# instance-based-loc/instance-based-loc

Hardware: AMD Instinct MI355X
Metric: query-frames localized/sec (embed+match+register) (higher is better)
Workload: dtype f16 (ViT MFMA operands, f32 accumulate) / f32+f64 (match, registration); 1 GPU; T: dinov2_vitb14 crops 224^2 (Q=7), 10000-instance memory (E=4), FPFH+RANSAC+coloured ICP on 5000-pt clouds, whole-memory evaluate; synthetic objects of extent U[0.15, 0.6] m on a 2.50 m grid (SURVEY 8d's U[0.2, 1.5] m re-scoped: its 5 000 points are too sparse to survive the radius-outlier removal); memory_instances=10000, points_per_object=5000, resident_feature_bytes_per_point=264, parallelism=frames-dp1+memory-replicated

## Files before the change

### instance-based-loc_amd/csrc/reg_api.hip

```cpp
#pragma clang fp contract(off)
#include <hip/hip_runtime.h>

#include <hipcub/hipcub.hpp>

#include <cctype>
#include <climits>
#include <cmath>
#include <cstdlib>
#include <cstring>
#include <string>
#include <vector>

#include "ibloc.h"
#include "reg_common.h"

#ifndef KNN_CELLS_NORMAL
#define KNN_CELLS_NORMAL 3.0
#endif
#ifndef KNN_CELLS_FEATURE
#define KNN_CELLS_FEATURE 5.0
#endif

#ifndef KNN_TILE_NORMAL
#define KNN_TILE_NORMAL 4
#endif
#ifndef KNN_TILE_FEATURE
#define KNN_TILE_FEATURE 2
#endif

int ibl_launch_normals(ibl_reg_ctx* ctx, const BatchGrid& g, const float4* pts, const int* seg_off, int n, double radius, int max_nn, float4* normals,
                       int* status, hipStream_t s);
int ibl_launch_fpfh(ibl_reg_ctx* ctx, const BatchGrid& g, const float4* pts, const float4* normals, const int* seg_off, int n, double radius, int max_nn,
                    unsigned char* spfh, int* nbr_idx, float* nbr_d2, int* nbr_cnt, float* fpfh, int matching_order, int* status,
                    hipStream_t s);
int ibl_launch_radius_count(const BatchGrid& g, const float4* pts, const int* seg_off, int n, double radius, int nb_points,
                            unsigned char* keep, hipStream_t s);

bool ibl_normals_fpfh_fusable(const ibl_reg_ctx* ctx, double radius_normal, int max_nn_normal, double radius_feature, int max_nn_feature);
int ibl_launch_normals_fpfh(ibl_reg_ctx* ctx, const BatchGrid& g, const float4* pts, const int* seg_off, int n, double radius_normal,
                            int max_nn_normal, double radius_feature, int max_nn_feature, float4* normals, unsigned char* spfh, int* nbr_idx,
                            float* nbr_d2, int* nbr_cnt, float* fpfh, int matching_order, int* status, hipStream_t s);
int ibl_launch_color_grad(ibl_reg_ctx* ctx, const BatchGrid& g, const float4* pts, const float4* normals, const int* seg_off, int q0, int q1, double radius,
                          int max_nn, float4* grad, int* status, hipStream_t s);

static int ibl_bbox_to_host(ibl_reg_ctx* ctx, const float4* P, const int* seg_off_dev, int n_seg, float* bbox_host, hipStream_t s) {
    if (n_seg <= 0) return IBL_OK;
    ArenaMark m(ctx);
    float* bbox;
    IBL_ARENA(bbox, float, (int64_t)n_seg * 6 + 6);
    int st = ibl_launch_bbox(P, seg_off_dev, n_seg, bbox, s);
    if (st) return st;
    IBL_HIP_CHECK(hipMemcpyAsync(bbox_host, bbox, sizeof(float) * 6 * (size_t)n_seg, hipMemcpyDeviceToHost, s));
    IBL_HIP_CHECK(hipStreamSynchronize(s));
    return IBL_OK;
}

struct DiagSwitch {
    const char* name;
    int RegDiag::*field;
    int lo = INT_MIN, hi = INT_MAX;
    bool auto0 = false;
};
static const DiagSwitch DIAG_SWITCHES[] = {
    {"knn_safety", nullptr},
    {"knn_rho", &RegDiag::knn_rho, 1, 4},
    {"knn_noguess", &RegDiag::knn_noguess},
    {"knn_debug", &RegDiag::knn_debug},
    {"feat_unfused", &RegDiag::feat_unfused},
    {"feat_valu", &RegDiag::feat_valu},
    {"feat_cand_cap", &RegDiag::feat_cand_cap, 1, INT_MAX, true},
    {"feat_p1_stride", &RegDiag::feat_p1_stride, 1},
    {"spfh_f64", &RegDiag::spfh_f64},
    {"spfh_qcap", &RegDiag::spfh_qcap, 1, INT_MAX, true},
    {"spfh_stats", &RegDiag::spfh_stats},
    {"eval_fullscan", &RegDiag::eval_fullscan},
    {"timing", &RegDiag::timing},
};

static const DiagSwitch* find_diag(const char* name) {
    for (const DiagSwitch& d : DIAG_SWITCHES)
        if (name && strcmp(name, d.name) == 0) return &d;
    return nullptr;
}

extern "C" int ibl_reg_ctx_set_diag(ibl_reg_ctx* ctx, const char* name, double value) {
    const DiagSwitch* d = find_diag(name);
    if (!ctx || !d || !std::isfinite(value)) return ibl_set_error(IBL_ERR_ARG, "ibl_reg_ctx_set_diag: null context, unknown switch or non-finite value");
    if (!d->field) ctx->diag.knn_safety = value;
    else if (d->auto0 && value == 0) ctx->diag.*d->field = 0;
    else ctx->diag.*d->field = (int)std::min(std::max(value, (double)d->lo), (double)d->hi);
    return IBL_OK;
}

extern "C" int ibl_reg_ctx_get_diag(const ibl_reg_ctx* ctx, const char* name, double* value) {
    const DiagSwitch* d = find_diag(name);
    if (!ctx || !d || !value) return ibl_set_error(IBL_ERR_ARG, "ibl_reg_ctx_get_diag: null argument or unknown switch");
    *value = d->field ? (double)(ctx->diag.*d->field) : ctx->diag.knn_safety;
    return IBL_OK;
}

extern "C" int ibl_reg_ctx_create(ibl_reg_ctx** out, int64_t arena_bytes) {
    if (!out || arena_bytes < (1 << 20)) return ibl_set_error(IBL_ERR_ARG, "ibl_reg_ctx_create: bad argument");
    ibl_reg_ctx* c = new ibl_reg_ctx();
    IBL_HIP_CHECK(hipGetDevice(&c->device));
    hipError_t e = hipMalloc(reinterpret_cast<void**>(&c->base), (size_t)arena_bytes);
    if (e != hipSuccess) {
        delete c;
        return ibl_set_error(IBL_ERR_HIP, "ibl_reg_ctx_create: hipMalloc(%lld) failed: %s", (long long)arena_bytes, hipGetErrorString(e));
    }
    c->size = arena_bytes;
    c->d_status = reinterpret_cast<int*>(c->base);
    c->used = 256;
    e = hipMemset(c->base, 0, 256);
    if (e != hipSuccess) { (void)hipFree(c->base); delete c; return ibl_set_error(IBL_ERR_HIP, "ibl_reg_ctx_create: memset failed"); }
    c->pin_size = 32 << 20;
    if (hipHostMalloc(reinterpret_cast<void**>(&c->pin), (size_t)c->pin_size, hipHostMallocDefault) != hipSuccess) { c->pin = nullptr; c->pin_size = 0; }
    for (const DiagSwitch& d : DIAG_SWITCHES) {
        std::string var = "IBL_";
        for (const char* p = d.name; *p; ++p) var += (char)toupper((unsigned char)*p);
        if (const char* v = getenv(var.c_str())) (void)ibl_reg_ctx_set_diag(c, d.name, atof(v));
    }
    *out = c;
    return IBL_OK;
}

extern "C" int ibl_reg_ctx_destroy(ibl_reg_ctx* ctx) {
    if (!ctx) return IBL_OK;
    (void)hipFree(ctx->base);
    if (ctx->pin) (void)hipHostFree(ctx->pin);
    delete ctx;
    return IBL_OK;
}

extern "C" int ibl_reg_ctx_reset(ibl_reg_ctx* ctx) {
    if (!ctx) return ibl_set_error(IBL_ERR_ARG, "ibl_reg_ctx_reset: null context");
    ctx->used = 256;
    return IBL_OK;
}

extern "C" int64_t ibl_reg_ctx_high_water(const ibl_reg_ctx* ctx) { return ctx ? ctx->high_water : -1; }

extern "C" int ibl_reg_ctx_status(ibl_reg_ctx* ctx, int clear) {
    if (!ctx) return -1;
    int h = 0;
    if (hipMemcpy(&h, ctx->d_status, sizeof(int), hipMemcpyDeviceToHost) != hipSuccess) return -1;
    if (clear) (void)hipMemset(ctx->d_status, 0, sizeof(int));
    return h;
}

static int check_seg(const int32_t* seg_off_host, int n_seg, const char* who) {
    if (!seg_off_host || n_seg < 0) return ibl_set_error(IBL_ERR_ARG, "%s: bad segment table", who);
    if (seg_off_host[0] != 0) return ibl_set_error(IBL_ERR_ARG, "%s: seg_off[0] must be 0", who);
    for (int s = 0; s < n_seg; ++s)
        if (seg_off_host[s + 1] < seg_off_host[s]) return ibl_set_error(IBL_ERR_ARG, "%s: seg_off must be non-decreasing", who);
// ... 306 lines not shown
```

### instance-based-loc_amd/csrc/reg_common.h

```cpp
#pragma once
#include <hip/hip_runtime.h>

#include <cstdint>

#include "ibl_common.h"

struct SegGrid {
    float minx, miny, minz, inv;
    int nx, ny, nz;
    int cell_base;
};

struct BatchGrid {
    const SegGrid* seg;
    const int* cell_start;
    const float4* sorted_pts;
    const int* order;
    int n_seg;
    const int* tile_base;
    const int* tile_seg;
    int n_tiles;
    int ts;
};

#define FM_P1_STRIDE 2

struct RegDiag {
    double knn_safety = 1.1;
    int knn_rho = 3;
    int knn_noguess = 0, knn_debug = 0;
    int feat_unfused = 0, feat_valu = 0, feat_cand_cap = 0;
    int feat_p1_stride = FM_P1_STRIDE;
    int spfh_f64 = 0, spfh_qcap = 0, spfh_stats = 0;
    int eval_fullscan = 0;
    int timing = 0;
};

struct ibl_reg_ctx {
    RegDiag diag;
    unsigned char* base = nullptr;
    int64_t size = 0;
    int64_t used = 0;
    int64_t high_water = 0;
    int device = 0;
    int* d_status = nullptr;
    unsigned char* pin = nullptr;
    int64_t pin_size = 0;
    int64_t pin_used = 0;
};

int ibl_stage_upload(ibl_reg_ctx* ctx, void* dst_dev, const void* src_host, int64_t bytes, hipStream_t s);
static inline void ibl_stage_reset(ibl_reg_ctx* ctx) { ctx->pin_used = 0; }

struct ArenaMark {
    ibl_reg_ctx* ctx;
    int64_t mark;
    explicit ArenaMark(ibl_reg_ctx* c) : ctx(c), mark(c->used) {}
    ~ArenaMark() { ctx->used = mark; }
};

template <typename T>
static inline T* arena_alloc(ibl_reg_ctx* ctx, int64_t count, bool* ok) {
    int64_t bytes = ibl_align_up(count * (int64_t)sizeof(T), 256);
    if (bytes < 256) bytes = 256;
    if (ctx->used + bytes > ctx->size) {
        *ok = false;
        return nullptr;
    }
    T* p = reinterpret_cast<T*>(ctx->base + ctx->used);
    ctx->used += bytes;
    if (ctx->used > ctx->high_water) ctx->high_water = ctx->used;
    return p;
}

#define IBL_ARENA(ptr, type, count)                                                                  \
    do {                                                                                             \
        bool _ok = true;                                                                             \
        ptr = arena_alloc<type>(ctx, (count), &_ok);                                                 \
        if (!_ok)                                                                                    \
            return ibl_set_error(IBL_ERR_ARENA, "device arena exhausted (%lld of %lld bytes used, need %lld more) at %s:%d", \
                                 (long long)ctx->used, (long long)ctx->size,                         \
                                 (long long)((count) * (int64_t)sizeof(type)), __FILE__, __LINE__);  \
    } while (0)

#define IBL_ERR_ARENA (-5)
#define IBL_ERR_OVERFLOW (-6)

#define IBL_ST_GRID_OVERFLOW 1
#define IBL_ST_KNN_SLOWPATH 2
#define IBL_ST_FEAT_OVERFLOW 4
#define IBL_ST_RANSAC_OVERFLOW 8
#define IBL_ST_FEAT_REDONE 16
#define IBL_ST_RANSAC_REDONE 32

int ibl_build_batch_grid(ibl_reg_ctx* ctx, const float4* pts, const int* seg_off_dev, const int* seg_off_host, int n_seg,
                         float cell, int64_t max_cells, bool collapse, BatchGrid* out, hipStream_t s);
int ibl_build_batch_grid_bounded(ibl_reg_ctx* ctx, const float4* pts, const int* seg_off_dev, const int* seg_off_host, int n_seg,
                                 float cell, int64_t cells_bound, BatchGrid* out, hipStream_t s);
int ibl_build_tile_grid(ibl_reg_ctx* ctx, const float4* pts, const int* seg_off_dev, const int* seg_off_host, int n_seg,
                        const float* bbox_host, double radius, int max_nn, int ts, int64_t max_cells, BatchGrid* out, hipStream_t s);

int ibl_launch_bbox(const float4* pts, const int* seg_off_dev, int n_seg, float* bbox_dev, hipStream_t s);

struct FeatSources { const float4* normals[3]; const float* fpfh[3]; const float4* grad[3]; const unsigned short* split[3]; const float* norm[3]; };
struct FeatPair { int qkind, qsrc, qcnt, dkind, dsrc, dcnt, out, pad; };

int ibl_feat_search_mfma(ibl_reg_ctx* ctx, const FeatPair* d_pairs, int n_pairs, int max_q, const FeatSources& src, int* pair_idx,
                         float* pair_d2, const int* need_pos, const int* need_list, int out0, int64_t out_count, bool* overflow,
                         hipStream_t s);

int ibl_features_on_batch(ibl_reg_ctx* ctx, const float4* P, const int* seg_off_dev, const int* seg_off_host, int n_seg, const float* bbox_host, double voxel_size,
                          double grad_radius, int gq0, int gq1, float4* normals, float* fpfh, unsigned short* fpfh_split, float* fpfh_norm,
                          float4* grad, hipStream_t s);

#ifdef __HIPCC__
__device__ __constant__ const float FM_MU[33] = {87.f, 46.f, 101.f, 26.f, 28.f, 17.f, 26.f, 26.f, 17.f, 14.f, 21.f, 7.f, 14.f, 19.f, 7.f, 8.f, 14.f,
                                                 6.f,  8.f,  13.f,  6.f,  5.f,  11.f, 6.f,  5.f,  10.f, 6.f,  3.f,  7.f,  14.f, 3.f, 6.f,  14.f};
typedef __attribute__((ext_vector_type(8))) _Float16 fm_piece_t;
struct __attribute__((aligned(4))) ibl_u4_a4 { unsigned x, y, z, w; };
__device__ __forceinline__ float fm_centred_norm(const float* __restrict__ x) {
    float a = 0.0f;
    for (int k = 0; k < 33; ++k) { const float v = x[k] - FM_MU[k]; a = __builtin_fmaf(v, v, a); }
    return a;
}
__device__ __forceinline__ fm_piece_t fm_operand_piece(const float* x8, float a, int pc) {
    fm_piece_t r;
#pragma unroll
    for (int e = 0; e < 8; ++e) r[e] = (_Float16)0.0f;
    if (pc < 4) {
#pragma unroll
        for (int e = 0; e < 8; ++e) r[e] = (_Float16)(x8[e] - FM_MU[8 * pc + e]);
    } else if (pc == 4) {
        const float w = a * 0.125f;
        const _Float16 nh = (_Float16)w, nl = (_Float16)(w - (float)nh);
        const float cw = 1.0e-3f * a + 4.0e-3f;
        _Float16 cu = (_Float16)cw;
        if ((float)cu < cw) cu = __builtin_bit_cast(_Float16, (unsigned short)(__builtin_bit_cast(unsigned short, cu) + 1));
        r[0] = (_Float16)(x8[0] - FM_MU[32]);
        r[1] = (_Float16)8.0f; r[2] = (_Float16)8.0f; r[3] = nh; r[4] = nl; r[5] = cu;
    }
    return r;
}
__device__ __forceinline__ int seg_of(const int* __restrict__ seg_off, int n_seg, int i) {
    int lo = 0, hi = n_seg;
    while (hi - lo > 1) {
        int mid = (lo + hi) >> 1;
        if (seg_off[mid] <= i) lo = mid; else hi = mid;
    }
    return lo;
}

__device__ __forceinline__ int cell_clamp(float v, float mn, float inv, int n) {
    int c = (int)floorf((v - mn) * inv);
    return c < 0 ? 0 : (c >= n ? n - 1 : c);
}

__device__ __forceinline__ float dist2f(float ax, float ay, float az, float bx, float by, float bz) {
    const float dx = ax - bx, dy = ay - by, dz = az - bz;
    return __builtin_fmaf(dz, dz, __builtin_fmaf(dy, dy, dx * dx));
}

__device__ __forceinline__ double wave_sum_d(double v) {
#pragma unroll
    for (int off = 32; off >= 1; off >>= 1) v += __shfl_xor(v, off, 64);
    return v;
}
__device__ __forceinline__ int wave_sum_i(int v) {
#pragma unroll
    for (int off = 32; off >= 1; off >>= 1) v += __shfl_xor(v, off, 64);
    return v;
}

__device__ __forceinline__ void cross3d(const double* a, const double* b, double* o) {
    o[0] = a[1] * b[2] - a[2] * b[1]; o[1] = a[2] * b[0] - a[0] * b[2]; o[2] = a[0] * b[1] - a[1] * b[0];
}
__device__ __forceinline__ double dot3d(const double* a, const double* b) { return a[0] * b[0] + a[1] * b[1] + a[2] * b[2]; }

__device__ __forceinline__ void xform_d(const double* T, double x, double y, double z, double* o) {
    o[0] = T[0] * x + T[1] * y + T[2] * z + T[3];
    o[1] = T[4] * x + T[5] * y + T[6] * z + T[7];
    o[2] = T[8] * x + T[9] * y + T[10] * z + T[11];
}

__device__ __forceinline__ void philox4x32(unsigned c0, unsigned c1, unsigned c2, unsigned c3, unsigned k0, unsigned k1,
                                           unsigned* out) {
#pragma unroll
    for (int r = 0; r < 10; ++r) {
        const unsigned long long p0 = (unsigned long long)0xD2511F53u * c0, p1 = (unsigned long long)0xCD9E8D57u * c2;
        const unsigned n0 = (unsigned)(p1 >> 32) ^ c1 ^ k0, n1 = (unsigned)p1, n2 = (unsigned)(p0 >> 32) ^ c3 ^ k1, n3 = (unsigned)p0;
        c0 = n0; c1 = n1; c2 = n2; c3 = n3;
        k0 += 0x9E3779B9u; k1 += 0xBB67AE85u;
    }
// ... 94 lines not shown
```

### instance-based-loc_amd/csrc/reg_featnn.hip

```cpp
#pragma clang fp contract(off)
#include <hip/hip_runtime.h>

#include <algorithm>
#include <cstdio>
#include <cstdlib>
#include <type_traits>

#include "reg_common.h"

typedef __attribute__((ext_vector_type(8))) _Float16 fm_h16x8;
typedef __attribute__((ext_vector_type(16))) float fm_f32x16;

#ifndef FM_SUB
#define FM_SUB 1
#endif
#define FM_DT (32 * FM_SUB)
#define FM_ROWB 112
#define FM_C 1.0e-3f
#define FM_NS 8.0f
#ifndef FM_NQ
#define FM_NQ 2
#endif
#define FM_QUEUE 256

// ... 144 lines not shown
                ah[h][s3] = *reinterpret_cast<const fm_h16x8*>(T.rows + (32 * h + n) * FM_ROWB + 32 * s3 + 16 * kg);
#pragma unroll
        for (int h = 0; h < FM_SUB; ++h) {
        fm_f32x16 acc[FM_NQ];
#pragma unroll
        for (int u = 0; u < FM_NQ; ++u)
#pragma unroll
            for (int i = 0; i < 16; ++i) acc[u][i] = 0.0f;
#pragma unroll
        for (int s3 = 0; s3 < 3; ++s3) {
#pragma unroll
            for (int u = 0; u < FM_NQ; ++u) acc[u] = __builtin_amdgcn_mfma_f32_32x32x16_f16(ah[h][s3], qh[u][s3], acc[u], 0, 0, 0);
        }
#pragma unroll
        for (int u = 0; u < FM_NQ; ++u) {
            float gm[4];
#pragma unroll
            for (int g = 0; g < 4; ++g) gm[g] = fminf(fminf(acc[u][4 * g], acc[u][4 * g + 1]), fminf(acc[u][4 * g + 2], acc[u][4 * g + 3]));
            const float lowest = fminf(fminf(gm[0], gm[1]), fminf(gm[2], gm[3]));
            if (PASS == 1) {
                mup[u] = fminf(mup[u], lowest);
            } else if (__builtin_amdgcn_ballot_w64(lowest <= mup[u] && valid[u]) != 0ull) {
#pragma unroll
                for (int g = 0; g < 4; ++g) {
                    if (__builtin_amdgcn_ballot_w64(gm[g] <= mup[u] && valid[u]) == 0ull) continue;
#pragma unroll
                    for (int e = 0; e < 4; ++e) {
                        const int i = 4 * g + e;
                        const int row = c * FM_DT + 32 * h + 8 * g + 4 * kg + e;
                        const bool hit = valid[u] && acc[u][i] <= mup[u] && row < P.dcnt;
                        const unsigned long long m = __builtin_amdgcn_ballot_w64(hit);
                        if (m) {
                            if (hit) queue[wave][qcount + __popcll(m & ((1ull << lane) - 1ull))] = make_int2(qi[u], row);
                            qcount += __popcll(m);
                            if (qcount > FM_QUEUE - 64) flush();
                        }
                    }
                }
            }
        }
        }
        if (more) stash(tiles[(it + 1) & 1]);
        __syncthreads();
    }
    if (PASS == 1) {
#pragma unroll
        for (int u = 0; u < FM_NQ; ++u) {
            const float m2 = fminf(mup[u], __shfl_xor(mup[u], 32, 64));
            if (valid[u] && kg == 0) up[P.out + qi[u]] = m2;
        }
    } else {
        flush();
    }
}

__global__ __launch_bounds__(256) void ibl_feat_exact_kernel(const FeatPair* __restrict__ pairs, FeatSources src, const FmCand* __restrict__ cand,
                                                             const unsigned long long* __restrict__ n_cand, int cand_cap,
                                                             unsigned long long* __restrict__ best) {
    const int total = (int)min(*n_cand, (unsigned long long)cand_cap);
    for (int c = blockIdx.x * 256 + threadIdx.x; c < total; c += gridDim.x * 256) {
        const FmCand K = cand[c];
        const FeatPair P = pairs[K.pair];
        const float* __restrict__ q = src.fpfh[P.qkind] + ((int64_t)P.qsrc + K.qi) * 33;
        const float* __restrict__ t = src.fpfh[P.dkind] + ((int64_t)P.dsrc + K.t) * 33;
        float acc = 0.0f;
#pragma unroll
        for (int k = 0; k < 33; ++k) { const float d = q[k] - t[k]; acc = __builtin_fmaf(d, d, acc); }
        const unsigned long long key = ((unsigned long long)__float_as_uint(acc) << 32) | (unsigned)K.t;
        atomicMin(&best[P.out + K.qi], key);
    }
}

__global__ __launch_bounds__(256) void ibl_feat_finish_kernel(const unsigned long long* __restrict__ best, int64_t i0, int64_t n,
                                                              int* __restrict__ pair_idx, float* __restrict__ pair_d2,
                                                              const unsigned long long* __restrict__ n_cand, int cand_cap, int* __restrict__ status) {
    if (blockIdx.x == 0 && threadIdx.x == 0 && *n_cand > (unsigned long long)cand_cap) atomicOr(status, IBL_ST_FEAT_OVERFLOW);
    const int64_t i = i0 + (int64_t)blockIdx.x * 256 + threadIdx.x;
    if (i >= i0 + n) return;
    const unsigned long long k = best[i];
    if (k == 0xFFFFFFFFFFFFFFFFull) { pair_idx[i] = 0; pair_d2[i] = INFINITY; }
    else { pair_idx[i] = (int)(unsigned)(k & 0xFFFFFFFFull); pair_d2[i] = __uint_as_float((unsigned)(k >> 32)); }
}

int ibl_feat_search_mfma(ibl_reg_ctx* ctx, const FeatPair* d_pairs, int n_pairs, int max_q, const FeatSources& src, int* pair_idx,
                         float* pair_d2, const int* need_pos, const int* need_list, int out0, int64_t out_count, bool* overflow,
                         hipStream_t s) {
    *overflow = false;
    if (n_pairs <= 0 || out_count <= 0) return IBL_OK;
    if (n_pairs > 32768) { *overflow = true; return IBL_OK; }
    ArenaMark mark(ctx);
    int cand_cap = (int)std::min<int64_t>(out_count * 8 + 65536, (int64_t)1 << 27);
    if (ctx->diag.feat_cand_cap) cand_cap = ctx->diag.feat_cand_cap;
    float* up; FmCand* cand; unsigned long long* n_cand; unsigned long long* best;
    IBL_ARENA(up, float, out_count + 64);
    IBL_ARENA(cand, FmCand, cand_cap);
    IBL_ARENA(n_cand, unsigned long long, 32);
    IBL_ARENA(best, unsigned long long, out_count + 64);
    float* up0 = up - out0;
    unsigned long long* best0 = best - out0;
    IBL_HIP_CHECK(hipMemsetAsync(n_cand, 0, sizeof(unsigned long long), s));
    IBL_HIP_CHECK(hipMemsetAsync(best, 0xFF, sizeof(unsigned long long) * (size_t)out_count, s));
    const bool indexed = need_pos != nullptr;
    const int p1s = ctx->diag.feat_p1_stride;
    bool conv = false;
    for (int k = 0; k < 3; ++k) conv = conv || (src.fpfh[k] && !src.split[k]);
    for (int p0 = 0; p0 < n_pairs; p0 += 32768) {
        const unsigned np = (unsigned)std::min(32768, n_pairs - p0);
        const dim3 grid((max_q + 128 * FM_NQ - 1) / (128 * FM_NQ), np);
        auto passes = [&](auto cv) {
            constexpr bool CV = decltype(cv)::value;
            if (indexed) {
                hipLaunchKernelGGL((ibl_feat_mfma_kernel<1, true, CV>), grid, dim3(256), 0, s, d_pairs + p0, src, up0, cand, n_cand, cand_cap, need_pos, need_list, out0, p1s);
                hipLaunchKernelGGL((ibl_feat_mfma_kernel<2, true, CV>), grid, dim3(256), 0, s, d_pairs + p0, src, up0, cand, n_cand, cand_cap, need_pos, need_list, out0, 1);
            } else {
                hipLaunchKernelGGL((ibl_feat_mfma_kernel<1, false, CV>), grid, dim3(256), 0, s, d_pairs + p0, src, up0, cand, n_cand, cand_cap, need_pos, need_list, out0, p1s);
                hipLaunchKernelGGL((ibl_feat_mfma_kernel<2, false, CV>), grid, dim3(256), 0, s, d_pairs + p0, src, up0, cand, n_cand, cand_cap, need_pos, need_list, out0, 1);
            }
        };
        if (conv) passes(std::true_type{});
        else passes(std::false_type{});
        IBL_LAUNCH_CHECK();
    }
    if (ctx->diag.timing >= 2) {
        unsigned long long h = 0;
        const hipError_t e = hipMemcpy(&h, n_cand, sizeof(h), hipMemcpyDeviceToHost);
        fprintf(stderr, "[reg-dbg] mfma passes done: %s; candidates %llu of cap %d, out_count %lld, pairs %d, max_q %d\n", hipGetErrorString(e), h, cand_cap,
                (long long)out_count, n_pairs, max_q);
    }
    hipLaunchKernelGGL(ibl_feat_exact_kernel, dim3(2048), dim3(256), 0, s, d_pairs, src, cand, n_cand, cand_cap, best0);
    IBL_LAUNCH_CHECK();
    hipLaunchKernelGGL(ibl_feat_finish_kernel, dim3((unsigned)((out_count + 255) / 256)), dim3(256), 0, s, best0, (int64_t)out0, out_count,
                       pair_idx, pair_d2, n_cand, cand_cap, ctx->d_status);
    IBL_LAUNCH_CHECK();
    return IBL_OK;
}
```

### instance-based-loc_amd/csrc/reg_match.hip

```cpp
#pragma clang fp contract(off)
#include <hip/hip_runtime.h>

#include <hipcub/hipcub.hpp>

#include <algorithm>
#include <array>
#include <cmath>
#include <cstdlib>
#include <map>
#include <vector>

#include "ibloc.h"
#include "reg_common.h"
#include "reg_stages.h"

#define FEATCOPY_GRAD 4

__global__ __launch_bounds__(256) void ibl_group_gather_kernel(const GroupDesc* __restrict__ groups, int G, const float4* __restrict__ det,
                                                               const int* __restrict__ det_off, const float4* __restrict__ mem,
                                                               const int* __restrict__ mem_off, const int* __restrict__ grp_off,
                                                               float4* __restrict__ out) {
    const int n = grp_off[G];
    const int i = blockIdx.x * 256 + threadIdx.x;
    if (i >= n) return;
// ... 419 lines not shown
    const float Rf = nextafterf((float)R, INFINITY);
    for (size_t p0 = 0; p0 < near.size(); p0 += 32768) {
        const unsigned np = (unsigned)std::min<size_t>(32768, near.size() - p0);
        hipLaunchKernelGGL(ibl_near_pair_kernel, dim3(NEAR_SPLIT, np), dim3(256), 0, s, d_near + p0, ps.det, ps.call->det.off_dev, ps.mem,
                           ps.call->mem.off_dev, Rf * Rf * 1.000001f, d_flags + p0);
        IBL_LAUNCH_CHECK();
    }
    IBL_HIP_CHECK(hipMemcpyAsync(ps.plan.near_flag.data(), d_flags, sizeof(int) * near.size(), hipMemcpyDeviceToHost, s));
    IBL_HIP_CHECK(hipStreamSynchronize(s));
    return IBL_OK;
}

static int recompute_groups(ibl_reg_ctx* ctx, RegPass& ps, const HostTables& h, double grad_radius, FeatSources* src) {
    const MatchPlan& plan = ps.plan;
    const RegCall& c = *ps.call;
    hipStream_t s = ps.s;
    const int G = (int)plan.groups.size(), Nd = plan.grp_off[G];
    GroupDesc* d_groups; int* d_grp_off; float4 *Pd, *normals_d, *grad_d; float *fpfh_d, *norm_d; unsigned short* split_d;
    IBL_ARENA(d_groups, GroupDesc, G);
    IBL_ARENA(d_grp_off, int, G + 1);
    IBL_ARENA(Pd, float4, Nd + 1);
    IBL_ARENA(normals_d, float4, Nd + 1);
    IBL_ARENA(grad_d, float4, Nd + 1);
    IBL_ARENA(fpfh_d, float, (int64_t)Nd * 33 + 64);
    IBL_ARENA(split_d, unsigned short, (int64_t)Nd * 48 + 64);
    IBL_ARENA(norm_d, float, (int64_t)Nd + 64);
    int st = ibl_stage_upload(ctx, d_groups, plan.groups.data(), sizeof(GroupDesc) * (int64_t)G, s);
    if (st) return st;
    st = ibl_stage_upload(ctx, d_grp_off, plan.grp_off.data(), sizeof(int) * (int64_t)(G + 1), s);
    if (st) return st;
    hipLaunchKernelGGL(ibl_group_gather_kernel, dim3((Nd + 255) / 256), dim3(256), 0, s, d_groups, G, ps.det, c.det.off_dev, ps.mem,
                       c.mem.off_dev, d_grp_off, Pd);
    IBL_LAUNCH_CHECK();
    const std::vector<float> grp_bbox = group_boxes(h, plan);
    st = ibl_features_on_batch(ctx, Pd, d_grp_off, plan.grp_off.data(), G, grp_bbox.empty() ? nullptr : grp_bbox.data(), c.params.voxel_size, grad_radius,
                               plan.grp_off[plan.G0], Nd, normals_d, fpfh_d, split_d, norm_d, grad_d, s);
    if (st) return st;
    src->normals[2] = normals_d; src->fpfh[2] = fpfh_d; src->grad[2] = grad_d; src->split[2] = split_d; src->norm[2] = norm_d;
    return IBL_OK;
}

static int assemble_features(ibl_reg_ctx* ctx, RegPass& ps, const FeatSources& src) {
    const std::vector<FeatCopy>& copies = ps.plan.copies;
    FeatCopy* d_copies;
    IBL_ARENA(d_copies, FeatCopy, (int64_t)copies.size());
    const int st = ibl_stage_upload(ctx, d_copies, copies.data(), sizeof(FeatCopy) * (int64_t)copies.size(), ps.s);
    if (st) return st;
    for (size_t c0 = 0; c0 < copies.size(); c0 += 32768) {
        const unsigned nc = (unsigned)std::min<size_t>(32768, copies.size() - c0);
        hipLaunchKernelGGL(ibl_feat_assemble_kernel, dim3(8, nc), dim3(256), 0, ps.s, d_copies + c0, src, ps.normals, (float*)nullptr, ps.grad);
        IBL_LAUNCH_CHECK();
    }
    return IBL_OK;
}

static int search_needed_targets(ibl_reg_ctx* ctx, RegPass& ps, const FeatSources& src, const MatchDev& d, bool use_mfma) {
    const MatchPlan& plan = ps.plan;
    hipStream_t s = ps.s;
    const int J = ps.J, Ns = ps.Ns, n_pairs0 = plan.n_pairs0, max_q = plan.max_q;
    const int64_t pts0 = plan.pts0;
    const int n1 = (int)(plan.pair_pts - pts0);
    const int n_pairs1 = (int)plan.pairs.size() - n_pairs0;
    if (!(n1 > 0 && n_pairs1 > 0 && Ns > 0)) return IBL_OK;
    int *need, *need_pos, *need_list;
    IBL_ARENA(need, int, (int64_t)n1 + 1);
    IBL_ARENA(need_pos, int, (int64_t)n1 + 1);
    IBL_ARENA(need_list, int, (int64_t)n1 + 1);
    IBL_HIP_CHECK(hipMemsetAsync(need, 0, sizeof(int) * ((size_t)n1 + 1), s));
    IBL_HIP_CHECK(hipMemsetD32Async((hipDeviceptr_t)(d.pair_d2 + pts0), 0x7f800000, (size_t)n1, s));
    IBL_HIP_CHECK(hipMemsetAsync(d.pair_idx + pts0, 0, sizeof(int) * (size_t)n1, s));
    hipLaunchKernelGGL(ibl_feat_need_kernel, dim3((Ns + 255) / 256), dim3(256), 0, s, d.d_sides, d.d_pairs, ps.d_job_off, J, d.nn, (int)pts0, need);
    IBL_LAUNCH_CHECK();
    size_t tmp_bytes = 0;
    IBL_HIP_CHECK(hipcub::DeviceScan::ExclusiveSum(nullptr, tmp_bytes, need, need_pos, n1 + 1, s));
    unsigned char* tmp;
    IBL_ARENA(tmp, unsigned char, (int64_t)tmp_bytes + 256);
    IBL_HIP_CHECK(hipcub::DeviceScan::ExclusiveSum(tmp, tmp_bytes, need, need_pos, n1 + 1, s));
    hipLaunchKernelGGL(ibl_feat_need_list_kernel, dim3((n1 + 255) / 256), dim3(256), 0, s, need, need_pos, n1, need_list);
    IBL_LAUNCH_CHECK();
    ps.dbg("need list");
    bool over = !use_mfma;
    if (use_mfma) {
        const int st = ibl_feat_search_mfma(ctx, d.d_pairs + n_pairs0, n_pairs1, max_q, src, d.pair_idx, d.pair_d2, need_pos, need_list, (int)pts0, n1,
                                            &over, s);
        if (st) return st;
    }
    for (int p0 = 0; over && p0 < n_pairs1; p0 += 32768) {
        const unsigned np = (unsigned)std::min(32768, n_pairs1 - p0);
        hipLaunchKernelGGL(ibl_feat_pair_nn_kernel<true>, dim3((max_q + 255) / 256, np), dim3(256), 0, s, d.d_pairs + n_pairs0 + p0, src,
                           d.pair_idx, d.pair_d2, need_pos, need_list, (int)pts0);
        IBL_LAUNCH_CHECK();
    }
    return IBL_OK;
}

static int search_features(ibl_reg_ctx* ctx, RegPass& ps, const FeatSources& src, const MatchDev& d) {
    const MatchPlan& plan = ps.plan;
    hipStream_t s = ps.s;
    const int J = ps.J, N = ps.N, Ns = ps.Ns, n_pairs0 = plan.n_pairs0, max_q = plan.max_q;
    int st = ibl_stage_upload(ctx, d.d_sides, plan.sides.data(), sizeof(SidePairs) * (int64_t)plan.sides.size(), s);
    if (st) return st;
    if (plan.pairs.empty() || N <= 0) {
        if (N > 0) IBL_HIP_CHECK(hipMemsetAsync(d.nn, 0, sizeof(int) * (size_t)N, s));
        return IBL_OK;
    }
    st = ibl_stage_upload(ctx, d.d_pairs, plan.pairs.data(), sizeof(FeatPair) * (int64_t)plan.pairs.size(), s);
    if (st) return st;
    const bool use_mfma = !ctx->diag.feat_valu && !ps.opt.force_valu;
    bool over = !use_mfma;
    ps.dbg("plan uploads");
    if (use_mfma) {
        st = ibl_feat_search_mfma(ctx, d.d_pairs, n_pairs0, max_q, src, d.pair_idx, d.pair_d2, nullptr, nullptr, 0, plan.pts0, &over, s);
        if (st) return st;
    }
    ps.dbg("forward search");
    for (int p0 = 0; over && p0 < n_pairs0; p0 += 32768) {
        const unsigned np = (unsigned)std::min(32768, n_pairs0 - p0);
        hipLaunchKernelGGL(ibl_feat_pair_nn_kernel<false>, dim3((max_q + 255) / 256, np), dim3(256), 0, s, d.d_pairs + p0, src, d.pair_idx,
                           d.pair_d2, (const int*)nullptr, (const int*)nullptr, 0);
        IBL_LAUNCH_CHECK();
    }
    if (Ns > 0) {
        hipLaunchKernelGGL(ibl_feat_fold_kernel, dim3((Ns + 255) / 256), dim3(256), 0, s, d.d_sides, d.d_pairs, d.pair_idx, d.pair_d2, ps.d_job_off,
                           J, 0, Ns, d.nn);
        IBL_LAUNCH_CHECK();
    }
    ps.dbg("forward fold");
    st = search_needed_targets(ctx, ps, src, d, use_mfma);
    if (st) return st;
    ps.dbg("reverse search");
    if (N > Ns) {
        hipLaunchKernelGGL(ibl_feat_fold_kernel, dim3((N - Ns + 255) / 256), dim3(256), 0, s, d.d_sides, d.d_pairs, d.pair_idx, d.pair_d2, ps.d_job_off,
                           J, Ns, N, d.nn);
        IBL_LAUNCH_CHECK();
    }
    ps.dbg("reverse fold");
    return IBL_OK;
}

static int features_and_search(ibl_reg_ctx* ctx, RegPass& ps, const HostTables& h, double grad_radius, const MatchDev& d) {
    const RegCall& c = *ps.call;
    ArenaMark md(ctx);
    FeatSources src{};
    const ibl_instance_features* feat[2] = {c.det.features, c.mem.features};
    for (int pl = 0; pl < 2; ++pl)
        if (feat[pl]) {
            src.normals[pl] = reinterpret_cast<const float4*>(feat[pl]->normals4);
            src.fpfh[pl] = feat[pl]->fpfh;
            src.split[pl] = feat[pl]->fpfh_split;
            src.norm[pl] = feat[pl]->fpfh_norm;
            src.grad[pl] = reinterpret_cast<const float4*>(feat[pl]->grad4);
        }
    int st;
    if (ps.plan.grp_off.back() > 0) {
        st = recompute_groups(ctx, ps, h, grad_radius, &src);
        if (st) return st;
    }
    if (!ps.plan.copies.empty()) {
        st = assemble_features(ctx, ps, src);
        if (st) return st;
    }
    ps.phase("recomputed groups + assemble");
    double fl = 0;
    for (int j = 0; j < ps.J; ++j)
        fl += 4.0 * 33.0 * (double)(ps.job_off[j + 1] - ps.job_off[j]) * (double)(ps.job_off[ps.J + j + 1] - ps.job_off[ps.J + j]);
    ibl_prof_begin(IBL_PROF_ST_FEATMATCH, fl, ps.s, &ps.tok_match);
    return search_features(ctx, ps, src, d);
}

int ibl_reg_match_stage(ibl_reg_ctx* ctx, RegPass& ps) {
    const RegCall& c = *ps.call;
    MatchPlan& plan = ps.plan;
    ArenaMark m2(ctx);
    MatchDev d = {};
    IBL_ARENA(d.nn, int, ps.N + 64);
    const double grad_radius = ps.max_dist_icp * 2.0;
    int st = check_instance_features(c, grad_radius);
    if (st) return st;
    const HostTables h = {ps.J, ps.jobs.data(), ps.job_off.data(), {c.det.off_host, c.mem.off_host},
                          {c.det.features ? c.det.features->bbox : nullptr, c.mem.features ? c.mem.features->bbox : nullptr}};
    const double rn = c.params.voxel_size * 2, rf = c.params.voxel_size * 5;
    const double R = std::max(2 * rf + rn, grad_radius + rn) * 1.001 + 1e-4;
    list_near_candidates(h, R, &plan);
    st = test_near_pairs(ctx, ps, R);
    if (st) return st;
    ps.phase("near-pair test");
    plan_feature_reuse(h, &plan);
    if (c.out.reuse_stats) for (int i = 0; i < 4; ++i) c.out.reuse_stats[i] = plan.reuse_stats[i];
    st = plan_feature_pairs(h, &plan);
    if (st) return st;
    if (c.out.reuse_stats) for (int i = 4; i < 6; ++i) c.out.reuse_stats[i] = plan.reuse_stats[i];
    ps.phase("host plan");
    IBL_ARENA(d.d_sides, SidePairs, 2 * ps.J);
    IBL_ARENA(d.d_pairs, FeatPair, (int64_t)plan.pairs.size() + 1);
    IBL_ARENA(d.pair_idx, int, plan.pair_pts + 64);
// ... 10 lines not shown
```

### instance-based-loc_amd/csrc/reg_stages.h

```cpp
#pragma once
#include <algorithm>
#include <array>
#include <map>
#include <vector>

#include "ibloc.h"
#include "reg_common.h"

#define ICP_BPJ 8

struct RegCall {
    ibl_cloud_pool det, mem;
    const int32_t* job_src_seg; const int32_t* job_tgt_seg;
    const uint32_t* job_ids;
    int n_jobs;
    ibl_register_params params;
    ibl_register_out out;
    hipStream_t stream;
};
struct RegPassOpts {
    bool force_valu = false;
    bool ransac_full_list = false;
};

struct JobDesc {
    int src_seg[3];
    int tgt_seg[3];
};
struct GroupDesc { int pool; int seg[3]; };
struct FeatCopy { int dst, src, count, kind; };
struct NearPair { int pool, a, b, pad; float boxa[6], boxb[6]; };
struct SidePairs { int qcnt[3]; int dcnt[3]; int pair[3][3]; };

struct RansacState {
    double best_T[16];
    double best_fit, best_rmse;
    long long est_k, next_i, walked, validated, last_update;
    int best_inl;
    int done;
    unsigned job_id;
    int pad_;
};
struct IcpState {
    double T[16];
    double fitness, rmse;
    int iter, done, started;
};

struct HostTables { int J; const JobDesc* jobs; const int* job_off; const int* off[2]; const float* bbox[2]; };
struct SlotPlan { int dst, count, pool, seg, grp, pos, side, kind, src; };
struct MatchPlan {
    std::vector<NearPair> near;
    std::map<std::array<int, 3>, int> near_id;
    std::vector<int> near_flag;
    std::vector<SlotPlan> slots;
    std::vector<GroupDesc> groups;
    std::vector<int> grp_off;
    int G0 = 0;
    std::vector<FeatCopy> copies;
    std::vector<FeatPair> pairs;
    std::vector<SidePairs> sides;
    int64_t pair_pts = 0, pts0 = 0;
    int n_pairs0 = 0, max_q = 1;
    int64_t reuse_stats[6] = {0, 0, 0, 0, 0, 0};
};

static inline void union_of_boxes(const int* segs, int only, const int* off, const float* boxes, float* lo, float* hi) {
    bool any = false;
    for (int c = 0; c < 3; ++c) lo[c] = hi[c] = 0.0f;
    for (int t = 0; t < 3; ++t) {
        if (only >= 0 && t != only) continue;
        if (segs[t] < 0 || off[segs[t] + 1] == off[segs[t]]) continue;
        const float* b = boxes + 6 * (size_t)segs[t];
        for (int c = 0; c < 3; ++c) { lo[c] = any ? std::min(lo[c], b[c]) : b[c]; hi[c] = any ? std::max(hi[c], b[3 + c]) : b[3 + c]; }
        any = true;
    }
}

struct RegPass {
    const RegCall* call;
    RegPassOpts opt;
    hipStream_t s;
    int J, N, Ns;
    bool colored;
    double max_dist_icp;
    std::vector<JobDesc> jobs;
    std::vector<int> job_off;
    MatchPlan plan;
    const float4 *det, *mem;
    JobDesc* d_jobs; int* d_job_off; int* d_piece_off; double* d_means;
    float4 *P, *normals, *grad;
    BatchGrid gC;
    int2* corr; int* n_corr;
    RansacState* rs;
    IcpState* is;
    void *tok_match, *tok_ransac, *tok_icp;
    int timing;
    double t_prev;
    void phase(const char* what);
    void dbg(const char* what) const;
};

int ibl_reg_match_stage(ibl_reg_ctx* ctx, RegPass& ps);
int ibl_reg_ransac_stage(ibl_reg_ctx* ctx, RegPass& ps);
int ibl_reg_icp_stage(ibl_reg_ctx* ctx, RegPass& ps);
```

Before: 840.3 query-frames/s.

## Tighten feature-search pass-2 bounds with per-side min across pairs

```diff
diff --git a/instance-based-loc_amd/csrc/reg_api.hip b/instance-based-loc_amd/csrc/reg_api.hip
--- a/instance-based-loc_amd/csrc/reg_api.hip
+++ b/instance-based-loc_amd/csrc/reg_api.hip
@@ -70,6 +70,7 @@
     {"feat_valu", &RegDiag::feat_valu},
     {"feat_cand_cap", &RegDiag::feat_cand_cap, 1, INT_MAX, true},
     {"feat_p1_stride", &RegDiag::feat_p1_stride, 1},
+    {"feat_pair_bounds", &RegDiag::feat_pair_bounds},
     {"spfh_f64", &RegDiag::spfh_f64},
     {"spfh_qcap", &RegDiag::spfh_qcap, 1, INT_MAX, true},
     {"spfh_stats", &RegDiag::spfh_stats},
diff --git a/instance-based-loc_amd/csrc/reg_common.h b/instance-based-loc_amd/csrc/reg_common.h
--- a/instance-based-loc_amd/csrc/reg_common.h
+++ b/instance-based-loc_amd/csrc/reg_common.h
@@ -31,6 +31,7 @@
     int knn_noguess = 0, knn_debug = 0;
     int feat_unfused = 0, feat_valu = 0, feat_cand_cap = 0;
     int feat_p1_stride = FM_P1_STRIDE;
+    int feat_pair_bounds = 0;
     int spfh_f64 = 0, spfh_qcap = 0, spfh_stats = 0;
     int eval_fullscan = 0;
     int timing = 0;
@@ -104,10 +105,12 @@
 
 struct FeatSources { const float4* normals[3]; const float* fpfh[3]; const float4* grad[3]; const unsigned short* split[3]; const float* norm[3]; };
 struct FeatPair { int qkind, qsrc, qcnt, dkind, dsrc, dcnt, out, pad; };
+struct SidePairs { int qcnt[3]; int dcnt[3]; int pair[3][3]; };
+struct FeatBounds { const SidePairs* sides; const int* job_off; int n_sides, n_pts; };
 
 int ibl_feat_search_mfma(ibl_reg_ctx* ctx, const FeatPair* d_pairs, int n_pairs, int max_q, const FeatSources& src, int* pair_idx,
-                         float* pair_d2, const int* need_pos, const int* need_list, int out0, int64_t out_count, bool* overflow,
-                         hipStream_t s);
+                         float* pair_d2, const int* need_pos, const int* need_list, int out0, int64_t out_count, const FeatBounds* bounds,
+                         bool* overflow, hipStream_t s);
 
 int ibl_features_on_batch(ibl_reg_ctx* ctx, const float4* P, const int* seg_off_dev, const int* seg_off_host, int n_seg, const float* bbox_host, double voxel_size,
                           double grad_radius, int gq0, int gq1, float4* normals, float* fpfh, unsigned short* fpfh_split, float* fpfh_norm,
diff --git a/instance-based-loc_amd/csrc/reg_featnn.hip b/instance-based-loc_amd/csrc/reg_featnn.hip
--- a/instance-based-loc_amd/csrc/reg_featnn.hip
+++ b/instance-based-loc_amd/csrc/reg_featnn.hip
@@ -250,17 +250,41 @@
     else { pair_idx[i] = (int)(unsigned)(k & 0xFFFFFFFFull); pair_d2[i] = __uint_as_float((unsigned)(k >> 32)); }
 }
 
+__global__ __launch_bounds__(256) void ibl_feat_side_bound_kernel(const SidePairs* __restrict__ sides, const FeatPair* __restrict__ pairs,
+                                                                  const int* __restrict__ job_off, int n_sides, const float* __restrict__ up,
+                                                                  unsigned* __restrict__ up2) {
+    const int i = blockIdx.x * 256 + threadIdx.x;
+    if (i >= job_off[n_sides]) return;
+    const int sgi = seg_of(job_off, n_sides, i);
+    const SidePairs S = sides[sgi];
+    int local = i - job_off[sgi], a = 0;
+    while (a < 2 && local >= S.qcnt[a]) { local -= S.qcnt[a]; ++a; }
+    float ub = INFINITY;
+#pragma unroll
+    for (int b = 0; b < 3; ++b) {
+        const int p = S.pair[a][b];
+        if (p >= 0) ub = fminf(ub, up[pairs[p].out + local]);
+    }
+#pragma unroll
+    for (int b = 0; b < 3; ++b) {
+        const int p = S.pair[a][b];
+        if (p >= 0) atomicMax(&up2[pairs[p].out + local], __float_as_uint(ub));
+    }
+}
+
 int ibl_feat_search_mfma(ibl_reg_ctx* ctx, const FeatPair* d_pairs, int n_pairs, int max_q, const FeatSources& src, int* pair_idx,
-                         float* pair_d2, const int* need_pos, const int* need_list, int out0, int64_t out_count, bool* overflow,
-                         hipStream_t s) {
+                         float* pair_d2, const int* need_pos, const int* need_list, int out0, int64_t out_count, const FeatBounds* bounds,
+                         bool* overflow, hipStream_t s) {
     *overflow = false;
     if (n_pairs <= 0 || out_count <= 0) return IBL_OK;
     if (n_pairs > 32768) { *overflow = true; return IBL_OK; }
     ArenaMark mark(ctx);
     int cand_cap = (int)std::min<int64_t>(out_count * 8 + 65536, (int64_t)1 << 27);
     if (ctx->diag.feat_cand_cap) cand_cap = ctx->diag.feat_cand_cap;
-    float* up; FmCand* cand; unsigned long long* n_cand; unsigned long long* best;
+    const bool tighten = bounds && bounds->n_pts > 0;
+    float* up; unsigned* up2 = nullptr; FmCand* cand; unsigned long long* n_cand; unsigned long long* best;
     IBL_ARENA(up, float, out_count + 64);
+    if (tighten) IBL_ARENA(up2, unsigned, out_count + 64);
     IBL_ARENA(cand, FmCand, cand_cap);
     IBL_ARENA(n_cand, unsigned long long, 32);
     IBL_ARENA(best, unsigned long long, out_count + 64);
@@ -268,27 +292,31 @@
     unsigned long long* best0 = best - out0;
     IBL_HIP_CHECK(hipMemsetAsync(n_cand, 0, sizeof(unsigned long long), s));
     IBL_HIP_CHECK(hipMemsetAsync(best, 0xFF, sizeof(unsigned long long) * (size_t)out_count, s));
+    if (tighten) IBL_HIP_CHECK(hipMemsetAsync(up2, 0, sizeof(unsigned) * (size_t)out_count, s));
     const bool indexed = need_pos != nullptr;
     const int p1s = ctx->diag.feat_p1_stride;
     bool conv = false;
     for (int k = 0; k < 3; ++k) conv = conv || (src.fpfh[k] && !src.split[k]);
-    for (int p0 = 0; p0 < n_pairs; p0 += 32768) {
-        const unsigned np = (unsigned)std::min(32768, n_pairs - p0);
-        const dim3 grid((max_q + 128 * FM_NQ - 1) / (128 * FM_NQ), np);
-        auto passes = [&](auto cv) {
-            constexpr bool CV = decltype(cv)::value;
-            if (indexed) {
-                hipLaunchKernelGGL((ibl_feat_mfma_kernel<1, true, CV>), grid, dim3(256), 0, s, d_pairs + p0, src, up0, cand, n_cand, cand_cap, need_pos, need_list, out0, p1s);
-                hipLaunchKernelGGL((ibl_feat_mfma_kernel<2, true, CV>), grid, dim3(256), 0, s, d_pairs + p0, src, up0, cand, n_cand, cand_cap, need_pos, need_list, out0, 1);
-            } else {
-                hipLaunchKernelGGL((ibl_feat_mfma_kernel<1, false, CV>), grid, dim3(256), 0, s, d_pairs + p0, src, up0, cand, n_cand, cand_cap, need_pos, need_list, out0, p1s);
-                hipLaunchKernelGGL((ibl_feat_mfma_kernel<2, false, CV>), grid, dim3(256), 0, s, d_pairs + p0, src, up0, cand, n_cand, cand_cap, need_pos, need_list, out0, 1);
-            }
-        };
-        if (conv) passes(std::true_type{});
-        else passes(std::false_type{});
+    const dim3 grid((max_q + 128 * FM_NQ - 1) / (128 * FM_NQ), (unsigned)n_pairs);
+    auto pass = [&](auto pv, auto iv, auto cv, float* bound0, int cstride) {
+        hipLaunchKernelGGL((ibl_feat_mfma_kernel<decltype(pv)::value, decltype(iv)::value, decltype(cv)::value>), grid, dim3(256), 0, s, d_pairs, src,
+                           bound0, cand, n_cand, cand_cap, need_pos, need_list, out0, cstride);
+    };
+    auto pass_of = [&](auto pv, float* bound0, int cstride) {
+        if (indexed) { if (conv) pass(pv, std::true_type{}, std::true_type{}, bound0, cstride); else pass(pv, std::true_type{}, std::false_type{}, bound0, cstride); }
+        else { if (conv) pass(pv, std::false_type{}, std::true_type{}, bound0, cstride); else pass(pv, std::false_type{}, std::false_type{}, bound0, cstride); }
+    };
+    pass_of(std::integral_constant<int, 1>{}, up0, p1s);
+    IBL_LAUNCH_CHECK();
+    float* bound0 = up0;
+    if (tighten) {
+        hipLaunchKernelGGL(ibl_feat_side_bound_kernel, dim3((bounds->n_pts + 255) / 256), dim3(256), 0, s, bounds->sides, d_pairs, bounds->job_off,
+                           bounds->n_sides, up0, up2 - out0);
         IBL_LAUNCH_CHECK();
-    }
+        bound0 = reinterpret_cast<float*>(up2) - out0;
+    }
+    pass_of(std::integral_constant<int, 2>{}, bound0, 1);
+    IBL_LAUNCH_CHECK();
     if (ctx->diag.timing >= 2) {
         unsigned long long h = 0;
         const hipError_t e = hipMemcpy(&h, n_cand, sizeof(h), hipMemcpyDeviceToHost);
diff --git a/instance-based-loc_amd/csrc/reg_match.hip b/instance-based-loc_amd/csrc/reg_match.hip
--- a/instance-based-loc_amd/csrc/reg_match.hip
+++ b/instance-based-loc_amd/csrc/reg_match.hip
@@ -525,7 +525,7 @@
     bool over = !use_mfma;
     if (use_mfma) {
         const int st = ibl_feat_search_mfma(ctx, d.d_pairs + n_pairs0, n_pairs1, max_q, src, d.pair_idx, d.pair_d2, need_pos, need_list, (int)pts0, n1,
-                                            &over, s);
+                                            nullptr, &over, s);
         if (st) return st;
     }
     for (int p0 = 0; over && p0 < n_pairs1; p0 += 32768) {
@@ -553,7 +553,9 @@
     bool over = !use_mfma;
     ps.dbg("plan uploads");
     if (use_mfma) {
-        st = ibl_feat_search_mfma(ctx, d.d_pairs, n_pairs0, max_q, src, d.pair_idx, d.pair_d2, nullptr, nullptr, 0, plan.pts0, &over, s);
+        const FeatBounds by_side = {d.d_sides, ps.d_job_off, J, Ns};
+        st = ibl_feat_search_mfma(ctx, d.d_pairs, n_pairs0, max_q, src, d.pair_idx, d.pair_d2, nullptr, nullptr, 0, plan.pts0,
+                                  ctx->diag.feat_pair_bounds ? nullptr : &by_side, &over, s);
         if (st) return st;
     }
     ps.dbg("forward search");
diff --git a/instance-based-loc_amd/csrc/reg_stages.h b/instance-based-loc_amd/csrc/reg_stages.h
--- a/instance-based-loc_amd/csrc/reg_stages.h
+++ b/instance-based-loc_amd/csrc/reg_stages.h
@@ -30,7 +30,6 @@
 struct GroupDesc { int pool; int seg[3]; };
 struct FeatCopy { int dst, src, count, kind; };
 struct NearPair { int pool, a, b, pad; float boxa[6], boxb[6]; };
-struct SidePairs { int qcnt[3]; int dcnt[3]; int pair[3][3]; };
 
 struct RansacState {
     double best_T[16];
```

Result: no change. 843.6 query-frames/s, median of 2 (+0.4%).
